# LahiruCooray/rl-aerial-manipulator

Hardware: AMD Instinct MI355X
Metric: env-steps/sec (whole node), hexacopter+arm waypoint task at 4096 envs/GPU (higher is better)
Workload: dtype f32

## Files before the change

### rl-aerial-manipulator_amd/csrc/amenv_capi.hip

```cpp
#include <hip/hip_runtime.h>
#include <hip/hip_ext.h>

#include <algorithm>
#include <cmath>
#include <cstdio>
#include <cstdlib>
#include <cstring>
#include <mutex>
#include <new>
#include <string>
#include <vector>

#include "amenv_kernels.hpp"
#include "amenv_team.hpp"
#include "amenv_team_host.hpp"
#include "amenv_quad.hpp"
#include "amenv_team_policy.hpp"
#include "amenv_quad_policy.hpp"
#include "amenv_lane_policy.hpp"
#include "amenv_rigid_policy.hpp"
#include "amenv_obsnorm.hpp"
#include "amenv_policy.hpp"
#include "amenv_train.hpp"
#include "amenv_mlp_train.hpp"
// ... 10 lines not shown
  TwoWave,
};

struct amenv {
  amenv_config cfg;
  int device = -1;
  int obs_dim = 20, act_dim = kActDim, nf = 0;
  void* blob = nullptr;
  unsigned long long* stats = nullptr;
  size_t blob_bytes = 0, fbytes = 0, ibytes = 0;
  uint32_t tile_bytes = 0;
  int n_tiles = 0;
  int block = 64;
  StepFamily family = StepFamily::Lane;
  void* team_consts = nullptr;
  uint32_t* pol_pack = nullptr;
  int pub_nj = 0;
  float* io_act = nullptr;
  float* io_obs = nullptr;
  float* io_term = nullptr;
  uint64_t steps = 0;
  bool dr = false;
  DrRanges dr_r = {{1.0f, 1.0f, 1.0f}, {0.0f, 0.0f, 0.0f}};
  bool lag = false;
  double lag_a[2] = {1.0, 1.0};
  void* lag_w = nullptr;
  hipEvent_t ev_start = nullptr, ev_stop = nullptr;
  std::string err;
  std::string kname;
};
// ... 334 lines not shown
  const amenv_config& c = e.cfg;
  const char* t = c.dtype == AMENV_F64 ? "double" : "float";
  const int nrot = (c.vehicle.n_rotors == 4 || c.vehicle.n_rotors == 6) ? c.vehicle.n_rotors : AMENV_MAX_ROTORS;
  const int kw = is_v1(&c) ? 2 : (c.task.num_waypoints == 1 ? 1 : AMENV_MAX_WAYPOINTS);
  char buf[200] = "";
  switch (e.family) {
    case StepFamily::Lane:
      std::snprintf(buf, sizeof(buf), "step_kernel<%s,NROT=%d,KW=%d,%s> block=%d", t, nrot, kw, c.vehicle.n_joints ? "v2+arm3" : (is_v1(&c) ? "v1" : "v2"), e.block); break;
    case StepFamily::LaneHelper:
      std::snprintf(buf, sizeof(buf), "step_kernel_pw<%s,NROT=%d,KW=%d,%s> (main wave + reset wave [+ observation wave + Monitor wave] per 64-env tile)", t, nrot, kw,
                    is_v1(&c) ? "v1" : "v2"); break;
    case StepFamily::Quad:
      std::snprintf(buf, sizeof(buf), "step_kernel_quad<NROT=%d,v2> (4 lanes per env, 16 envs per wave + episode-end helper wave)", c.vehicle.n_rotors); break;
    case StepFamily::Team:
      std::snprintf(buf, sizeof(buf), "step_kernel_team<%s,NROT=6,v2+arm3> (16 lanes per env: 4 RK4 stages x 4 components, 4 envs per wave + %s)", t,
                    team_wide(e) ? "one episode-end helper wave per 4" : "episode-end helper wave"); break;
    case StepFamily::Staged:
      std::snprintf(buf, sizeof(buf), "step_kernel_armk<%s,NROT=6> block=320 (4 RK4 stage waves + main wave per 64-env tile)", t); break;
    case StepFamily::TwoWave:
      std::snprintf(buf, sizeof(buf), "step_kernel_arm2w<float,NROT=6> block=128 (2 waves per 64-env tile)"); break;
  }
  std::string name = buf;
  if (e.dr) name += " +dr";
  if (e.lag) name += " +lag";
  if (e.pub_nj == 1 || e.pub_nj == 2) name += " [" + std::to_string(e.pub_nj) + "-joint arm: phantom links inside, pack / unpack at the C ABI]";
  return name;
}

template <typename... P, typename... A>
hipError_t launch(const amenv& e, bool timed, void (*k)(P...), dim3 grid, dim3 block, size_t lds, hipStream_t s, A... args) {
  if (timed) hipExtLaunchKernelGGL(k, grid, block, lds, s, e.ev_start, e.ev_stop, 0, args...);
// ... 32 lines not shown
hipError_t launch_step(const amenv& e, const StepIO& io, int T_steps, hipStream_t s, bool timed) {
  if (T_steps > 0) return launch_rollout<T, NROT, KW, VAR, NJ, DR, LAG>(e, io, T_steps, s);
  ArmArg<T, NJ> AA;
  if constexpr (NJ > 0) AA.p = make_arm<T>(e); else AA.unused = 0;
  const HotParams<T, NROT> P = make_hot<T, NROT>(e);
  const ColdParams C = make_cold(e);
  const StepTail tl{io.terminal_obs, io.ep_return, io.ep_len, io.stats};
  const uint32_t tb = e.tile_bytes;
  const int32_t n = e.cfg.num_envs;
  switch (e.family) {
    case StepFamily::Team:
      if constexpr (NJ == 3 && !DR) {
        const TeamParamsT<T> TP = make_team<T>(e);
        if (team_wide(e))
          return launch(e, timed, step_kernel_team<T, NROT, 4>, dim3(e.n_tiles * 4), dim3(320), 0, s, e.blob, n, int32_t(e.n_tiles * 4),
                        reinterpret_cast<const float*>(io.actions), TP.consts, io.obs, static_cast<T*>(io.reward), io.done, io.info, tl, C);
        return launch(e, timed, step_kernel_team<T, NROT, 1>, dim3(e.n_tiles * 16), dim3(128), 0, s, e.blob, n, int32_t(e.n_tiles * 16),
                      reinterpret_cast<const float*>(io.actions), TP.consts, io.obs, static_cast<T*>(io.reward), io.done, io.info, tl, C);
      }
      break;
    case StepFamily::Staged:
      if constexpr (NJ == 3 && !DR) {
        if constexpr (sizeof(T) == 8) {
          hipError_t ea = hipFuncSetAttribute(reinterpret_cast<const void*>(&step_kernel_armk<T, NROT>), hipFuncAttributeMaxDynamicSharedMemorySize, 96 * 1024);
          if (ea != hipSuccess) return ea;
        }
        const size_t lds = size_t(64 * ObsDim<VAR, NJ>::value + 12 * 64) * sizeof(float) + size_t((4 * kAggSlots + 6) * 64) * sizeof(T);
        return launch(e, timed, step_kernel_armk<T, NROT>, dim3(e.n_tiles), dim3(320), lds, s, e.blob, tb, n, io.actions, io.obs, io.reward, io.done, io.info, tl, P, C, AA);
      }
      break;
    case StepFamily::TwoWave:
      if constexpr (NJ == 3 && sizeof(T) == 4 && !DR) {
        const size_t lds = size_t(64 * ObsDim<VAR, NJ>::value + (kArmXchgSlots + 12) * 64) * sizeof(float);
// ... 59 lines not shown
}

template <typename T>
hipError_t launch_observe(const amenv& e, float* obs, float* ee, hipStream_t s) {
  const int n = e.cfg.num_envs, bs = 256, K = e.cfg.task.num_waypoints, nj = e.cfg.vehicle.n_joints;
  if (obs) hipLaunchKernelGGL((observe_kernel<T>), dim3((n + bs - 1) / bs), dim3(bs), 0, s, n, K, e.cfg.task.variant, nj, e.cfg.task.ee_task, e.tile_bytes, make_arm<T>(e),
                              (const void*)e.blob, obs);
  if (ee) hipLaunchKernelGGL((ee_position_kernel<T>), dim3((n + bs - 1) / bs), dim3(bs), 0, s, n, K, nj, e.tile_bytes, make_arm<T>(e), (const void*)e.blob, ee);
  return hipGetLastError();
}

template <typename T>
hipError_t launch_transpose(const amenv& e, void* f, int32_t* i, int to_api, hipStream_t s) {
  const int bs = 256, n = e.cfg.num_envs;
  hipLaunchKernelGGL((transpose_state_kernel<T>), dim3((n + bs - 1) / bs), dim3(bs), 0, s, n, e.nf, e.cfg.task.num_waypoints, e.pub_nj , e.tile_bytes, e.blob, (T*)f, i, to_api);
  return hipGetLastError();
}

bool aligned16(const void* p) { return (reinterpret_cast<uintptr_t>(p) & 15u) == 0; }

#ifndef AMENV_RIGID_WG16_MAX
#define AMENV_RIGID_WG16_MAX 6144
#endif
#ifndef AMENV_RIGID_WG64_MAX
#define AMENV_RIGID_WG64_MAX 24576
#endif
template <int NROT, int KW, int VAR, bool NORM, bool DR, bool LAG>
hipError_t launch_rigid_policy_k(const amenv& e, int T, const PolicyIO& io, const NormArg& N, hipStream_t s) {
  const HotParams<float, NROT> HP = make_hot<float, NROT>(e);
  const ColdParams C = make_cold(e);
// ... 270 lines not shown
  };
  DeviceGuard g(device);
  hipError_t s;
  if ((s = hipMalloc(&e->blob, e->blob_bytes)) != hipSuccess ||
      (s = hipMalloc((void**)&e->stats, sizeof(unsigned long long) * kStatsWords)) != hipSuccess ||
      (s = hipMemset(e->blob, 0, e->blob_bytes)) != hipSuccess ||
      (s = hipMemset(e->stats, 0, sizeof(unsigned long long) * kStatsWords)) != hipSuccess ||
      (s = (cfg->dtype == AMENV_F64 ? launch_reset<double>(*e, nullptr, nullptr, 1, nullptr) : launch_reset<float>(*e, nullptr, nullptr, 1, nullptr))) != hipSuccess ||
      (s = hipDeviceSynchronize()) != hipSuccess)
    return alloc_failed("device allocation failed", s);
  const bool quad = quad_ok(*cfg), team = team_ok(*cfg);
  if (rigid_pol_ok(*cfg) || arm_pol_ok(*cfg))
    if ((s = hipMalloc((void**)&e->pol_pack, size_t(kPolPackWords) * sizeof(uint32_t))) != hipSuccess) return alloc_failed("policy pack", s);
  if ((quad || team) && (s = upload_team_consts<float>(e, team)) != hipSuccess) return alloc_failed(quad ? "quad constants" : "team constants", s);
  if (family == StepFamily::Team && cfg->dtype == AMENV_F64 && (s = upload_team_consts<double>(e, true)) != hipSuccess) return alloc_failed("team constants (fp64)", s);
  if (e->pub_nj == 1 || e->pub_nj == 2) {
    if ((s = hipMalloc((void**)&e->io_act, n * 7 * sizeof(float))) != hipSuccess || (s = hipMalloc((void**)&e->io_obs, n * 29 * sizeof(float))) != hipSuccess ||
        (s = hipMalloc((void**)&e->io_term, n * 29 * sizeof(float))) != hipSuccess)
      return alloc_failed("n-link adapter buffers", s);
  }
  *out = e;
  return AMENV_OK;
}

int amenv_destroy(amenv* e) {
  if (!e) return AMENV_OK;
  {
    DeviceGuard g(e->device);
    if (e->blob) (void)hipFree(e->blob);
    if (e->stats) (void)hipFree(e->stats);
    if (e->team_consts) (void)hipFree(e->team_consts);
    if (e->pol_pack) (void)hipFree(e->pol_pack);
    if (e->lag_w) (void)hipFree(e->lag_w);
    if (e->io_act) (void)hipFree(e->io_act);
    if (e->io_obs) (void)hipFree(e->io_obs);
    if (e->io_term) (void)hipFree(e->io_term);
    if (e->ev_start) (void)hipEventDestroy(e->ev_start);
    if (e->ev_stop) (void)hipEventDestroy(e->ev_stop);
  }
  delete e;
  return AMENV_OK;
}

const char* amenv_last_error(const amenv* e) { return e ? e->err.c_str() : g_create_err.c_str(); }
const char* amenv_kernel_name(const amenv* e) { return e ? e->kname.c_str() : ""; }

// ... 1 lines not shown
hipError_t pad_actions(const amenv& e, const float* actions, hipStream_t s) {
  const int n = e.cfg.num_envs;
  hipLaunchKernelGGL(arm_pad_actions_kernel, dim3((n * 7 + 255) / 256), dim3(256), 0, s, actions, n, e.pub_nj, e.io_act);
  return hipGetLastError();
}
hipError_t cut_obs(const amenv& e, const float* rows29, const uint8_t* rows_of, float* out, hipStream_t s) {
  const int n = e.cfg.num_envs, od = 23 + 2 * e.pub_nj;
  hipLaunchKernelGGL(arm_cut_obs_kernel, dim3((n * od + 255) / 256), dim3(256), 0, s, rows29, n, e.pub_nj, rows_of, out);
  return hipGetLastError();
}
}

int amenv_set_seed(amenv* e, uint64_t seed) {
  if (!e) return AMENV_ERR_INVALID;
  e->cfg.seed = seed;
  return AMENV_OK;
}

int amenv_set_randomization(amenv* e, const amenv_randomization* r) {
  if (!e) return AMENV_ERR_INVALID;
  if (!r) {
    e->dr = false;
    e->dr_r = DrRanges{{1.0f, 1.0f, 1.0f}, {0.0f, 0.0f, 0.0f}};
    e->kname = kernel_name(*e);
    return AMENV_OK;
  }
  if (r->struct_size != sizeof(amenv_randomization)) return fail(e, AMENV_ERR_INVALID, "amenv_set_randomization: struct_size must be sizeof(amenv_randomization)");
  if (e->cfg.vehicle.n_joints > 0)
    return fail(e, AMENV_ERR_INVALID, "amenv_set_randomization: built for rigid vehicles (an arm vehicle's mass and inertia are not one scalar scale)");
  if (e->cfg.vehicle.n_rotors != 4 && e->cfg.vehicle.n_rotors != 6)
// ... 89 lines not shown
  if (!in) return fail(e, AMENV_ERR_INVALID, "amenv_set_rotor_state: NULL argument");
  if (!e->lag) return fail(e, AMENV_ERR_INVALID, "amenv_set_rotor_state: the rotor lag is off (amenv_set_rotor_lag)");
  DeviceGuard g(e->device);
  hipStream_t s = (hipStream_t)stream;
  AMENV_HIP(e, e->cfg.dtype == AMENV_F64 ? launch_lag_transpose<double>(*e, const_cast<void*>(in), 0, s) : launch_lag_transpose<float>(*e, const_cast<void*>(in), 0, s));
  return AMENV_OK;
}

int amenv_reset(amenv* e, const uint8_t* mask, float* obs_out, void* stream) {
  if (!e) return AMENV_ERR_INVALID;
  DeviceGuard g(e->device);
  hipStream_t s = (hipStream_t)stream;
  float* o = (e->io_obs && obs_out) ? e->io_obs : obs_out;
  AMENV_HIP(e, e->cfg.dtype == AMENV_F64 ? launch_reset<double>(*e, mask, o, 0, s) : launch_reset<float>(*e, mask, o, 0, s));
  if (e->lag) AMENV_HIP(e, e->cfg.dtype == AMENV_F64 ? launch_lag_reset<double>(*e, mask, s) : launch_lag_reset<float>(*e, mask, s));
  if (o != obs_out) AMENV_HIP(e, cut_obs(*e, e->io_obs, nullptr, obs_out, s));
  return AMENV_OK;
}

int amenv_observe(amenv* e, float* obs_out, void* stream) {
  if (!e || !obs_out) return fail(e, AMENV_ERR_INVALID, "amenv_observe: NULL argument");
  DeviceGuard g(e->device);
  hipStream_t s = (hipStream_t)stream;
  float* o = e->io_obs ? e->io_obs : obs_out;
  AMENV_HIP(e, e->cfg.dtype == AMENV_F64 ? launch_observe<double>(*e, o, nullptr, s) : launch_observe<float>(*e, o, nullptr, s));
  if (o != obs_out) AMENV_HIP(e, cut_obs(*e, e->io_obs, nullptr, obs_out, s));
  return AMENV_OK;
}

int amenv_ee_position(amenv* e, float* ee_out, void* stream) {
// ... 41 lines not shown
  return AMENV_OK;
}

int amenv_rollout(amenv* e, int32_t n_steps, const float* actions, float* obs, void* reward, uint8_t* done, uint32_t* info_bits,
                  void* stream) {
  if (!e) return AMENV_ERR_INVALID;
  if (n_steps <= 0 || !actions) return fail(e, AMENV_ERR_INVALID, "amenv_rollout: n_steps must be > 0 and actions non-NULL");
  if (!aligned16(actions) || (obs && !aligned16(obs))) return fail(e, AMENV_ERR_INVALID, "amenv_rollout: actions/obs must be 16-byte aligned");
  if (e->family == StepFamily::Team && e->cfg.dtype == AMENV_F64) return fail(e, AMENV_ERR_INVALID, "amenv_rollout: the fp64 lane-team build is a logic gate of amenv_step only");
  if (e->io_act) return fail(e, AMENV_ERR_INVALID, "amenv_rollout: arms with 1 or 2 joints are served through amenv_step (the adapters at the C ABI are per step)");
  DeviceGuard g(e->device);
  StepIO io{reinterpret_cast<const float4*>(actions), obs, reward, done, info_bits, nullptr, nullptr, nullptr, e->stats};
  hipStream_t s = (hipStream_t)stream;
  hipError_t st = e->cfg.dtype == AMENV_F64 ? dispatch_step<double>(*e, io, n_steps, s) : dispatch_step<float>(*e, io, n_steps, s);
  AMENV_HIP(e, st);
  e->steps += uint64_t(e->cfg.num_envs) * uint64_t(n_steps);
  return AMENV_OK;
}

int amenv_rollout_policy(amenv* e, int32_t n_steps, const float* flat_params, uint64_t seed, uint32_t draw0, float* obs, float* actions, float* logp,
                         float* values, float* rewards, uint8_t* dones, uint32_t* info_bits, float* terminal_obs, void* stream) {
  if (!e) return AMENV_ERR_INVALID;
  const bool quad = !e->dr && !e->lag && quad_ok(e->cfg), rigid = !quad && rigid_pol_ok(e->cfg);
  if (!quad && !rigid && !arm_pol_ok(e->cfg))
    return fail(e, AMENV_ERR_INVALID, "amenv_rollout_policy: built for fp32 vehicles: rigid with 4 or 6 rotors (every task), or the 6-rotor vehicle with a "
                "1..3-link arm (v2 task, 1..4 waypoints, any joint axes)");
  if (n_steps <= 0 || !flat_params || !obs || !actions || !logp || !values || !rewards || !dones)
    return fail(e, AMENV_ERR_INVALID, "amenv_rollout_policy: n_steps must be > 0 and flat_params / obs / actions / logp / values / rewards / dones non-NULL");
  if (rigid && (!aligned16(obs) || !aligned16(actions) || (terminal_obs && !aligned16(terminal_obs))))
    return fail(e, AMENV_ERR_INVALID, "amenv_rollout_policy: obs / actions / terminal_obs must be 16-byte aligned");
// ... 4 lines not shown
  if (quad) {
    const QuadParams QP = make_quad(*e);
    const dim3 gq(e->n_tiles * 4), bq(256);
    if (e->cfg.vehicle.n_rotors == 4) hipLaunchKernelGGL((rollout_policy_kernel_quad<4>), gq, bq, 0, s, e->blob, e->tile_bytes, n, (int)n_steps, io, e->stats, make_cold(*e), QP);
    else hipLaunchKernelGGL((rollout_policy_kernel_quad<6>), gq, bq, 0, s, e->blob, e->tile_bytes, n, (int)n_steps, io, e->stats, make_cold(*e), QP);
  } else if (rigid) {
    AMENV_HIP(e, launch_rigid_policy<false>(*e, (int)n_steps, io, NormArg{nullptr, 0.0f, 0.0, 0}, s));
  } else if (e->family == StepFamily::Team && !e->io_act) {
    const TeamParams TP = make_team<float>(*e);
    if (n <= 4096) hipLaunchKernelGGL((rollout_policy_kernel_team<6, 1>), dim3(e->n_tiles * 4), dim3(256), 0, s, e->blob, e->tile_bytes, n, (int)n_steps, io, e->stats, make_cold(*e), TP);
    else hipLaunchKernelGGL((rollout_policy_kernel_team<6, 2>), dim3(e->n_tiles * 4), dim3(256), 0, s, e->blob, e->tile_bytes, n, (int)n_steps, io, e->stats, make_cold(*e), TP);
  } else {
    AMENV_HIP(e, launch_lane_policy(*e, (int)n_steps, io, s));
  }
  AMENV_HIP(e, hipGetLastError());
  e->steps += uint64_t(e->cfg.num_envs) * uint64_t(n_steps);
  return AMENV_OK;
}

int amenv_get_state(amenv* e, void* fstate, int32_t* istate, void* stream) {
  if (!e) return AMENV_ERR_INVALID;
  DeviceGuard g(e->device);
  hipStream_t s = (hipStream_t)stream;
  AMENV_HIP(e, e->cfg.dtype == AMENV_F64 ? launch_transpose<double>(*e, fstate, istate, 1, s) : launch_transpose<float>(*e, fstate, istate, 1, s));
  return AMENV_OK;
}

int amenv_set_state(amenv* e, const void* fstate, const int32_t* istate, void* stream) {
  if (!e) return AMENV_ERR_INVALID;
  DeviceGuard g(e->device);
  hipStream_t s = (hipStream_t)stream;
  AMENV_HIP(e, e->cfg.dtype == AMENV_F64 ? launch_transpose<double>(*e, const_cast<void*>(fstate), const_cast<int32_t*>(istate), 0, s)
                                          : launch_transpose<float>(*e, const_cast<void*>(fstate), const_cast<int32_t*>(istate), 0, s));
  return AMENV_OK;
}

int amenv_stats_read(amenv* e, amenv_stats* out, int reset, void* stream) {
  if (!e || !out) return fail(e, AMENV_ERR_INVALID, "amenv_stats_read: NULL argument");
  DeviceGuard g(e->device);
  hipStream_t s = (hipStream_t)stream;
  static_assert(S_COUNT <= kStatsStride, "stats replica stride");
  std::vector<unsigned long long> rep(size_t(kStatsReplicas) * kStatsStride);
  AMENV_HIP(e, hipMemcpyAsync(rep.data(), e->stats, rep.size() * sizeof(unsigned long long), hipMemcpyDeviceToHost, s));
  if (reset) AMENV_HIP(e, hipMemsetAsync(e->stats, 0, rep.size() * sizeof(unsigned long long), s));
  AMENV_HIP(e, hipStreamSynchronize(s));
  unsigned long long h[S_COUNT] = {0};
  for (int r = 0; r < kStatsReplicas; r++)
    for (int k = 0; k < S_COUNT; k++) h[k] += rep[size_t(r) * kStatsStride + k];
// ... 391 lines not shown
```

### rl-aerial-manipulator_amd/csrc/amenv_team.hpp

```cpp
#pragma once
#include <type_traits>

#include "amenv_kernels.hpp"

#define AMENV_FN __device__ __forceinline__

namespace amenv_dev {

template <int CTRL> __device__ __forceinline__ float dpp_(float v) {
  return __builtin_bit_cast(float, __builtin_amdgcn_update_dpp(0, __builtin_bit_cast(int, v), CTRL, 0xF, 0xF, true));
}
template <int CTRL> __device__ __forceinline__ double dpp_(double v) {
  const int lo = __builtin_amdgcn_update_dpp(0, __double2loint(v), CTRL, 0xF, 0xF, true);
  const int hi = __builtin_amdgcn_update_dpp(0, __double2hiint(v), CTRL, 0xF, 0xF, true);
  return __hiloint2double(hi, lo);
}
template <int P0, int P1, int P2, int P3> __device__ __forceinline__ float qp(float v) { return dpp_<P0 | (P1 << 2) | (P2 << 4) | (P3 << 6)>(v); }
template <int P0, int P1, int P2, int P3> __device__ __forceinline__ double qp(double v) { return dpp_<P0 | (P1 << 2) | (P2 << 4) | (P3 << 6)>(v); }
template <int P0, int P1, int P2, int P3> __device__ __forceinline__ int qpi(int v) {
  return __builtin_amdgcn_update_dpp(0, v, P0 | (P1 << 2) | (P2 << 4) | (P3 << 6), 0xF, 0xF, true);
}
template <int N> __device__ __forceinline__ float row_ror(float v) { return dpp_<0x120 + N>(v); }
template <int N> __device__ __forceinline__ double row_ror(double v) { return dpp_<0x120 + N>(v); }
template <int N> __device__ __forceinline__ float row_shr(float v) { return dpp_<0x110 + N>(v); }
// ... 56 lines not shown
#pragma unroll
      for (int k = 0; k < NC4; k++) {
        const float4 v = tab[k * 16 + (lane & 15)];
        c[4 * k] = v.x; c[4 * k + 1] = v.y; c[4 * k + 2] = v.z; c[4 * k + 3] = v.w;
      }
    } else {
      const X* tab = static_cast<const X*>(table);
#pragma unroll
      for (int k = 0; k < NC4 * 4; k++) c[k] = tab[k * 16 + (lane & 15)];
    }
  }
};
using TeamLane = TeamLaneT<float>;

template <typename X>
__device__ __forceinline__ void team_load_issue(const char* tile, int i, const TeamLaneT<X>& L, TeamEnvT<X>& E) {
  constexpr uint32_t GB = 64u * 4u * sizeof(X);
  const uint32_t eoff = (uint32_t(i & 63) * 4u + uint32_t(L.cc)) * uint32_t(sizeof(X));
  auto gload = [&](int g) { return *reinterpret_cast<const X*>(tile + kIntBytes + uint32_t(g) * GB + eoff); };
  E.y = TeamStateT<X>{gload(0), gload(1), gload(2), gload(3), gload(5), gload(6)};
  E.WP = gload(4);
  const int4 iv = *(reinterpret_cast<const int4*>(tile) + (i & 63));
  E.step = iv.x; E.counter = iv.y; E.flags = iv.z; E.episode = iv.w;
}
template <typename X>
__device__ __forceinline__ void team_load_unpack(TeamEnvT<X>& E) {
  E.final_yaw = bc<3>(E.y.P); E.last_distance = bc<3>(E.y.V); E.ep_return = bc<3>(E.y.W);
}
template <typename X>
__device__ __forceinline__ void team_load(const char* tile, int i, const TeamLaneT<X>& L, TeamEnvT<X>& E) {
  team_load_issue(tile, i, L, E);
  team_load_unpack(E);
}

template <typename X>
__device__ __forceinline__ void team_store(char* tile, int i, const TeamLaneT<X>& L, const TeamEnvT<X>& E, bool store_wp = true) {
  constexpr uint32_t GB = 64u * 4u * sizeof(X);
  const uint32_t eoff = (uint32_t(i & 63) * 4u + uint32_t(L.cc)) * uint32_t(sizeof(X));
// ... 150 lines not shown
template <typename S> __device__ __forceinline__ S team_scalar_load(const void* p) {
  typedef const __attribute__((address_space(4))) uint32_t ConstWord;
  ConstWord* src = (ConstWord*)p;
  S v;
  uint32_t* dst = reinterpret_cast<uint32_t*>(&v);
  static_assert(sizeof(S) % 4 == 0, "copied word by word");
#pragma unroll
  for (int k = 0; k < int(sizeof(S) / 4); k++) dst[k] = src[k];
  return v;
}
template <typename X> __device__ __forceinline__ TeamParamsT<X> team_load_params(const void* block) {
  return team_scalar_load<TeamParamsT<X>>(static_cast<const char*>(block) + team_table_bytes<X>());
}
__device__ __forceinline__ const void* team_launder(const void* p) { asm volatile("" : "+s"(p)); return p; }

template <typename X> struct TeamStepLateArgs { float* obs; X* reward_out; uint8_t* done; uint32_t* info; StepTail tl; ColdParams C; };
struct TeamStepFirstArgs { void* blob; int32_t n_envs, n_blocks; const float* actions; const void* lane_consts; };
template <typename X> using TeamStepKernelFn = void (*)(decltype(TeamStepFirstArgs::blob), decltype(TeamStepFirstArgs::n_envs), decltype(TeamStepFirstArgs::n_blocks),
                                                        decltype(TeamStepFirstArgs::actions), decltype(TeamStepFirstArgs::lane_consts), decltype(TeamStepLateArgs<X>::obs),
                                                        decltype(TeamStepLateArgs<X>::reward_out), decltype(TeamStepLateArgs<X>::done), decltype(TeamStepLateArgs<X>::info),
                                                        decltype(TeamStepLateArgs<X>::tl), decltype(TeamStepLateArgs<X>::C));
template <typename X> __device__ __forceinline__ TeamStepLateArgs<X> team_late_args() {
  static_assert(sizeof(TeamStepFirstArgs) == 32 && alignof(TeamStepLateArgs<X>) == 8 && alignof(StepTail) == 8 && alignof(ColdParams) == 8,
                "TeamStepLateArgs mirrors the argument segment from byte 32 on");
  const void* ka = team_launder((const void*)__builtin_amdgcn_kernarg_segment_ptr());
  struct Head { float* obs; X* reward_out; uint8_t* done; uint32_t* info; StepTail tl; };
  static_assert(sizeof(Head) == offsetof(TeamStepLateArgs<X>, C), "the arguments in front of ColdParams");
  const Head h = team_scalar_load<Head>(static_cast<const char*>(ka) + sizeof(TeamStepFirstArgs));
  TeamStepLateArgs<X> a;
  a.obs = h.obs; a.reward_out = h.reward_out; a.done = h.done; a.info = h.info; a.tl = h.tl;
  return a;
}
template <typename X> __device__ __forceinline__ ColdParams team_late_cold() {
  const void* ka = team_launder((const void*)__builtin_amdgcn_kernarg_segment_ptr());
  return team_scalar_load<ColdParams>(static_cast<const char*>(ka) + sizeof(TeamStepFirstArgs) + offsetof(TeamStepLateArgs<X>, C));
}

template <typename X, int NROT, int MW>
__global__ __launch_bounds__(64 * (MW + 1)) void step_kernel_team(void* __restrict__ blob, int32_t n_envs, int32_t n_blocks, const float* __restrict__ actions,
                                                        const void* __restrict__ lane_consts, float* __restrict__ obs, X* __restrict__ reward_out,
                                                        uint8_t* __restrict__ done, uint32_t* __restrict__ info, const StepTail tl, const ColdParams C) {
  constexpr uint32_t tile_bytes = kIntBytes + 7u * 64u * 4u * uint32_t(sizeof(X));
  static_assert(NROT == 6, "team kernel: 6-rotor airframe");
  constexpr int AD = 7, OD = 29;
  __shared__ X rst[3][64];
  static_assert(MW == 1 || MW == 4, "one helper wave of 64 lanes = 16 quads serves at most four integrating waves");
  constexpr int ROWS = 4 * MW;
  __shared__ uint32_t fl[ROWS][4];
  __shared__ uint32_t have[ROWS];
  __shared__ unsigned long long acc[S_COUNT];
#ifdef AMENV_STAMPS
  unsigned long long stamps_[kStampSlots] = {0, 0, 0, 0, 0, 0, 0, 0};
#endif
  const int wave = __builtin_amdgcn_readfirstlane(int(threadIdx.x) >> 6);
  const int role = wave == MW ? 1 : 0;
  team_arg(blob, n_envs, n_blocks, actions, lane_consts);
  AMENV_STAMP(0);
  TeamLaneT<X> L;
  L.init_lane();
  const int row = role ? L.lane >> 2 : wave * 4 + (L.lane >> 4);
  const int i0 = (MW == 1 ? team_group_of_block(int(blockIdx.x), n_blocks) : team_group16_of_block(int(blockIdx.x), n_blocks)) * ROWS;
  const int i = i0 + row;
  const bool active = i < n_envs;
  char* tile = static_cast<char*>(blob) + size_t(i0 >> 6) * tile_bytes;
  TeamEnvT<X> E;
#ifdef AMENV_TEAM_DIAG_NOHELPER
  if (role == 1) { __syncthreads(); return; }
#endif
  if (role == 1) {
    {
      constexpr uint32_t GB = 64u * 4u * sizeof(X);
      const uint32_t eoff = (uint32_t(i & 63) * 4u + uint32_t(L.cc)) * uint32_t(sizeof(X));
      E.y.P = *reinterpret_cast<const X*>(tile + kIntBytes + eoff);
      E.y.V = *reinterpret_cast<const X*>(tile + kIntBytes + GB + eoff);
      const int4 iv = *(reinterpret_cast<const int4*>(tile) + (i & 63));
      E.step = iv.x; E.counter = iv.y; E.flags = iv.z; E.episode = iv.w;
    }
    const TeamParamsT<X> P = team_load_params<X>(team_launder(lane_consts));
    const X ce[3] = {L.cc == 0 ? X(1) : X(0), L.cc == 1 ? X(1) : X(0), L.cc == 2 ? X(1) : X(0)};
    static_assert(TC_E0 == 0 && TC_E1 == 1 && TC_E2 == 2, "ce[] stands in for c[] in team_reset_draw");
    const bool owned = n_blocks <= kStatsReplicas;
    if (L.lane < S_COUNT) acc[L.lane] = 0ull;
    const X dtc = P.h * X(P.substeps), slack = X(0.01) + X(50) * dtc * dtc;
    const X reach = fma_(dtc, abs_(E.y.V), abs_(E.y.P)) + slack;
    const bool lane_may = (L.cc < 3 && !(reach < X(5.7735))) || (L.cc == 2 && !(E.y.P - dtc * abs_(E.y.V) - slack > X(0.1)));
    const unsigned long long mm = __ballot(lane_may);
#ifdef AMENV_TEAM_DIAG_NOPREDICT
    constexpr bool kPredict = false;
#else
    constexpr bool kPredict = true;
#endif
    const bool serve = row < ROWS;
    const bool hlead = serve && L.cc == 0;
    const bool may = kPredict && serve && (((mm >> (L.lane & 60)) & 0xFull) != 0ull || E.step >= P.max_steps || ((E.flags & AMENV_FLAGBIT_FWR) && E.counter >= P.counter_limit) ||
                                  (P.flags & AMENV_FLAG_NAN_GUARD));
    if (hlead) have[row] = may ? 1u : 0u;
    unsigned long long* totals = tl.stats + size_t(blockIdx.x & (kStatsReplicas - 1)) * kStatsStride;
    unsigned long long mine = 0ull;
    bool fetched = false;
    if (__ballot(may) != 0ull) {
      if (owned && L.lane < S_COUNT) mine = totals[L.lane];
      fetched = true;
      if (may) {
        const TeamResetT<X> R = team_reset_draw<X>(C, ce, L.cc, E.episode, i);
        rst[0][L.lane] = R.P; rst[1][L.lane] = R.WP; rst[2][L.lane] = R.final_yaw;
      }
    }
    __syncthreads();
#ifdef AMENV_TEAM_DIAG_NOPOST
    return;
#endif
    const bool ended = hlead && (fl[hlead ? row : 0][0] & 1u) != 0;
    if (__ballot(ended) != 0ull) {
      if (!fetched && owned && L.lane < S_COUNT) mine = totals[L.lane];
      if (ended) {
        const uint32_t bits = fl[row][1];
        const int ep_len = int(fl[row][2]);
        const float ep_ret = __uint_as_float(fl[row][3]);
        if (tl.ep_return) tl.ep_return[i] = ep_ret;
        if (tl.ep_len) tl.ep_len[i] = ep_len;
        if (owned) accumulate_stats_lane(acc, 0, bits, ep_len, ep_ret);
        else accumulate_stats_lane(tl.stats, int(blockIdx.x), bits, ep_len, ep_ret);
      }
      if (owned) {
        __builtin_amdgcn_fence(__ATOMIC_ACQ_REL, "wavefront");
        __builtin_amdgcn_wave_barrier();
        if (L.lane < S_COUNT) totals[L.lane] = mine + acc[L.lane];
      }
    }
    return;
  }
#ifndef AMENV_TEAM_DIAG_NOPRIO
  __builtin_amdgcn_s_setprio(3);
#endif
  const int ia = active ? i : n_envs - 1;
  team_load_issue(tile, i, L, E);
  const float act_f = actions[size_t(ia) * AD + L.cc];
  const float actj_f = actions[size_t(ia) * AD + 4 + (L.cc < 3 ? L.cc : 2)];
  L.load_table(lane_consts);
  __builtin_amdgcn_sched_barrier(0);
  const TeamParamsT<X> P = team_load_params<X>(team_launder(lane_consts));
  const TeamStepLateArgs<X> A = team_late_args<X>();
  __builtin_amdgcn_sched_barrier(0);
  L.init_obs_cols();
  const ColdParams Cm{};
  team_load_unpack(E);
  const X act = X(act_f), actj = X(actj_f);
  const uint32_t obs_bytes = uint32_t(n_envs) * uint32_t(OD * 4);
  const uint32_t rowb = uint32_t(i) * uint32_t(OD * 4);
  uint32_t voA = L.okA ? rowb + L.offA * 4u : kOob, voB = L.okB ? rowb + L.offB * 4u : kOob, voC = L.okC ? rowb + L.offC * 4u : kOob;
  asm volatile("" : "+v"(voA), "+v"(voB), "+v"(voC));
  const __amdgpu_buffer_rsrc_t r_obs = team_rsrc(A.obs, obs_bytes), r_term = team_rsrc(A.tl.terminal_obs, A.tl.terminal_obs ? obs_bytes : 0u);
  uint32_t so1 = 0, so2 = 0, voR = kOob, voD = kOob;
  if constexpr (sizeof(X) == 4) {
    constexpr uint32_t GB = 64u * 4u * 4u;
    const uint32_t eoff = (uint32_t(i & 63) * 4u + uint32_t(L.cc)) * 4u;
    so1 = kIntBytes + uint32_t(L.bb) * GB + eoff;
    so2 = L.q2 ? eoff : kIntBytes + (L.q0 ? 5u : (L.q1 ? 6u : 4u)) * GB + eoff;
    voR = active && L.lead ? uint32_t(i) * 4u : kOob; voD = active && L.lead ? uint32_t(i) : kOob;
    asm volatile("" : "+v"(so1), "+v"(so2), "+v"(voR), "+v"(voD));
  }
  AMENV_STAMP(1);
  AMENV_STAMP_DRAIN();
  AMENV_STAMP(2);
  TeamOutT<X> o = team_advance<NROT, true>(P, Cm, L, E, act, actj, i, active, nullptr, nullptr, nullptr);
  const bool resets = o.ended && (P.flags & AMENV_FLAG_AUTO_RESET);
  if (L.lead) {
    fl[row][0] = (o.ended && active ? 1u : 0u) | (resets ? 2u : 0u);
    if (o.ended) { fl[row][1] = o.bits; fl[row][2] = uint32_t(o.ep_len); fl[row][3] = __float_as_uint(o.ep_ret); }
  }
  AMENV_STAMP(4);
#ifdef AMENV_STAMPS
  stamps_[3] = __ballot(o.ended && active) != 0ull ? 1ull : 0ull;
#endif
  __syncthreads();
  const bool any_end = __ballot(o.ended) != 0ull;
  const X tA = o.vA, tB = o.vB, tC = o.vC;
  if (any_end && resets) {
    TeamResetT<X> R;
    const int hl = row * 4 + L.cc;
    if (have[row]) R = TeamResetT<X>{rst[0][hl], rst[1][hl], rst[2][hl], X(0), X(0), X(0)};
    else R = team_reset_draw<X>(team_late_cold<X>(), L.c, L.cc, E.episode, i);
    team_apply_reset(L, team_reset_obs(P, L, R), E, o);
  }
  AMENV_STAMP(5);
  if constexpr (sizeof(X) == 4) {
    const __amdgpu_buffer_rsrc_t r_tile = team_rsrc(tile, tile_bytes);
    const bool l3 = L.cc == 3;
    const X g0 = sel(l3, E.final_yaw, E.y.P), g1 = sel(l3, E.last_distance, E.y.V), g3 = sel(l3, E.ep_return, E.y.W);
    const X sv = sel(L.q0, g0, sel(L.q1, g1, sel(L.q2, E.y.Q, g3)));
    __builtin_amdgcn_raw_buffer_store_b32(__float_as_int(sv), r_tile, int(so1), 0, 0);
    const int ival = sel(L.cc == 0, E.step, sel(L.cc == 1, E.counter, sel(L.cc == 2, E.flags, E.episode)));
    const float s2 = sel(L.q0, E.y.TH, sel(L.q1, E.y.THD, sel(L.q2, __int_as_float(ival), E.WP)));
    __builtin_amdgcn_raw_buffer_store_b32(__float_as_int(s2), r_tile, int(L.bb == 3 && !resets ? kOob : so2), 0, 0);
  } else {
    team_store(tile, i, L, E, resets);
  }
  __builtin_amdgcn_raw_buffer_store_b32(__float_as_int(float(o.vA)), r_obs, int(voA), 0, 0);
  __builtin_amdgcn_raw_buffer_store_b32(__float_as_int(float(o.vB)), r_obs, int(voB), 0, 0);
  __builtin_amdgcn_raw_buffer_store_b32(__float_as_int(float(o.vC)), r_obs, int(voC), 0, 0);
  if constexpr (sizeof(X) == 4) {
    const uint32_t nb = uint32_t(n_envs);
    __builtin_amdgcn_raw_buffer_store_b32(__float_as_int(o.reward), team_rsrc(A.reward_out, nb * 4u), int(voR), 0, 0);
    __builtin_amdgcn_raw_buffer_store_b8(uint8_t(o.ended ? 1 : 0), team_rsrc(A.done, nb), int(voD), 0, 0);
    __builtin_amdgcn_raw_buffer_store_b32(int(o.bits), team_rsrc(A.info, nb * 4u), int(voR), 0, 0);
  } else {
    if (active && L.lead) { A.reward_out[uint32_t(i)] = o.reward; A.done[uint32_t(i)] = o.ended ? 1 : 0; A.info[uint32_t(i)] = o.bits; }
  }
  if (any_end) {
    __builtin_amdgcn_raw_buffer_store_b32(__float_as_int(float(tA)), r_term, int(o.ended ? voA : kOob), 0, 0);
    __builtin_amdgcn_raw_buffer_store_b32(__float_as_int(float(tB)), r_term, int(o.ended ? voB : kOob), 0, 0);
    __builtin_amdgcn_raw_buffer_store_b32(__float_as_int(float(tC)), r_term, int(o.ended ? voC : kOob), 0, 0);
  }
  AMENV_STAMP(6);
#ifdef AMENV_STAMPS
  AMENV_STAMP_DRAIN();
  AMENV_STAMP(7);
  if (L.lane == 0 && blockIdx.x * MW + wave < kStampWaves)
    for (int kk = 0; kk < kStampSlots; kk++) A.tl.stats[kStampBase + (blockIdx.x * MW + wave) * kStampSlots + kk] = stamps_[kk];
#endif
}

static_assert(std::is_same<decltype(&step_kernel_team<float, 6, 4>), TeamStepKernelFn<float>>::value && std::is_same<decltype(&step_kernel_team<float, 6, 1>), TeamStepKernelFn<float>>::value &&
                  std::is_same<decltype(&step_kernel_team<double, 6, 4>), TeamStepKernelFn<double>>::value && std::is_same<decltype(&step_kernel_team<double, 6, 1>), TeamStepKernelFn<double>>::value,
              "step_kernel_team's parameters and TeamStepFirstArgs / TeamStepLateArgs have come apart");

template <int NROT>
// ... 30 lines not shown
```

Measured before the change: 945.3 million.

## Replace team helper-wave reset draws with a persistent reset-draw cache

Adds a per-env device cache of precomputed reset draws keyed by episode parity. The helper wave now only refills the next episode's entry when it is stale. The integrating waves read the cached draw instead of waiting at a __syncthreads for LDS results from the helper. Episode statistics and ep_return/ep_len writes move into the main waves as atomics. This removes the block barrier and the helper's predictive draw and stats work. In exchange it adds global cache traffic, refresh kernels and memsets after reset, step and state loads, and atomics on episode end.

```diff
diff --git a/rl-aerial-manipulator_amd/csrc/amenv_capi.hip b/rl-aerial-manipulator_amd/csrc/amenv_capi.hip
--- a/rl-aerial-manipulator_amd/csrc/amenv_capi.hip
+++ b/rl-aerial-manipulator_amd/csrc/amenv_capi.hip
@@ -48,6 +48,7 @@
   int block = 64;
   StepFamily family = StepFamily::Lane;
   void* team_consts = nullptr;
+  void* team_rcache = nullptr;
   uint32_t* pol_pack = nullptr;
   int pub_nj = 0;
   float* io_act = nullptr;
@@ -412,7 +413,7 @@
       std::snprintf(buf, sizeof(buf), "step_kernel_quad<NROT=%d,v2> (4 lanes per env, 16 envs per wave + episode-end helper wave)", c.vehicle.n_rotors); break;
     case StepFamily::Team:
       std::snprintf(buf, sizeof(buf), "step_kernel_team<%s,NROT=6,v2+arm3> (16 lanes per env: 4 RK4 stages x 4 components, 4 envs per wave + %s)", t,
-                    team_wide(e) ? "one episode-end helper wave per 4" : "episode-end helper wave"); break;
+                    team_wide(e) ? "one reset-cache keeper wave per 4" : "reset-cache keeper wave"); break;
     case StepFamily::Staged:
       std::snprintf(buf, sizeof(buf), "step_kernel_armk<%s,NROT=6> block=320 (4 RK4 stage waves + main wave per 64-env tile)", t); break;
     case StepFamily::TwoWave:
@@ -475,9 +476,9 @@
         const TeamParamsT<T> TP = make_team<T>(e);
         if (team_wide(e))
           return launch(e, timed, step_kernel_team<T, NROT, 4>, dim3(e.n_tiles * 4), dim3(320), 0, s, e.blob, n, int32_t(e.n_tiles * 4),
-                        reinterpret_cast<const float*>(io.actions), TP.consts, io.obs, static_cast<T*>(io.reward), io.done, io.info, tl, C);
+                        reinterpret_cast<const float*>(io.actions), TP.consts, e.team_rcache, io.obs, static_cast<T*>(io.reward), io.done, io.info, tl, C);
         return launch(e, timed, step_kernel_team<T, NROT, 1>, dim3(e.n_tiles * 16), dim3(128), 0, s, e.blob, n, int32_t(e.n_tiles * 16),
-                      reinterpret_cast<const float*>(io.actions), TP.consts, io.obs, static_cast<T*>(io.reward), io.done, io.info, tl, C);
+                      reinterpret_cast<const float*>(io.actions), TP.consts, e.team_rcache, io.obs, static_cast<T*>(io.reward), io.done, io.info, tl, C);
       }
       break;
     case StepFamily::Staged:
@@ -567,6 +568,18 @@
 hipError_t launch_transpose(const amenv& e, void* f, int32_t* i, int to_api, hipStream_t s) {
   const int bs = 256, n = e.cfg.num_envs;
   hipLaunchKernelGGL((transpose_state_kernel<T>), dim3((n + bs - 1) / bs), dim3(bs), 0, s, n, e.nf, e.cfg.task.num_waypoints, e.pub_nj , e.tile_bytes, e.blob, (T*)f, i, to_api);
+  return hipGetLastError();
+}
+
+hipError_t team_rcache_refresh(const amenv& e, hipStream_t s) {
+  if (!e.team_rcache) return hipSuccess;
+  const bool f64 = e.cfg.dtype == AMENV_F64;
+  const int n_pad = e.n_tiles * 64;
+  hipError_t st = hipMemsetAsync(e.team_rcache, kResetCacheStale, size_t(n_pad) * kResetCacheWords * (f64 ? 8 : 4), s);
+  if (st != hipSuccess) return st;
+  const dim3 grid((n_pad * 4 + 255) / 256), block(256);
+  if (f64) hipLaunchKernelGGL(team_rcache_fill_kernel<double>, grid, block, 0, s, (const void*)e.blob, e.tile_bytes, n_pad, static_cast<double*>(e.team_rcache), make_cold(e));
+  else hipLaunchKernelGGL(team_rcache_fill_kernel<float>, grid, block, 0, s, (const void*)e.blob, e.tile_bytes, n_pad, static_cast<float*>(e.team_rcache), make_cold(e));
   return hipGetLastError();
 }
 
@@ -867,6 +880,11 @@
     if ((s = hipMalloc((void**)&e->pol_pack, size_t(kPolPackWords) * sizeof(uint32_t))) != hipSuccess) return alloc_failed("policy pack", s);
   if ((quad || team) && (s = upload_team_consts<float>(e, team)) != hipSuccess) return alloc_failed(quad ? "quad constants" : "team constants", s);
   if (family == StepFamily::Team && cfg->dtype == AMENV_F64 && (s = upload_team_consts<double>(e, true)) != hipSuccess) return alloc_failed("team constants (fp64)", s);
+  if (family == StepFamily::Team) {
+    if ((s = hipMalloc(&e->team_rcache, size_t(e->n_tiles) * 64 * kResetCacheWords * ts)) != hipSuccess || (s = team_rcache_refresh(*e, nullptr)) != hipSuccess ||
+        (s = hipDeviceSynchronize()) != hipSuccess)
+      return alloc_failed("team reset-draw cache", s);
+  }
   if (e->pub_nj == 1 || e->pub_nj == 2) {
     if ((s = hipMalloc((void**)&e->io_act, n * 7 * sizeof(float))) != hipSuccess || (s = hipMalloc((void**)&e->io_obs, n * 29 * sizeof(float))) != hipSuccess ||
         (s = hipMalloc((void**)&e->io_term, n * 29 * sizeof(float))) != hipSuccess)
@@ -883,6 +901,7 @@
     if (e->blob) (void)hipFree(e->blob);
     if (e->stats) (void)hipFree(e->stats);
     if (e->team_consts) (void)hipFree(e->team_consts);
+    if (e->team_rcache) (void)hipFree(e->team_rcache);
     if (e->pol_pack) (void)hipFree(e->pol_pack);
     if (e->lag_w) (void)hipFree(e->lag_w);
     if (e->io_act) (void)hipFree(e->io_act);
@@ -914,6 +933,12 @@
 int amenv_set_seed(amenv* e, uint64_t seed) {
   if (!e) return AMENV_ERR_INVALID;
   e->cfg.seed = seed;
+  if (e->team_rcache) {
+    DeviceGuard g(e->device);
+    AMENV_HIP(e, hipDeviceSynchronize());
+    AMENV_HIP(e, hipMemset(e->team_rcache, kResetCacheStale, size_t(e->n_tiles) * 64 * kResetCacheWords * (e->cfg.dtype == AMENV_F64 ? 8 : 4)));
+    AMENV_HIP(e, hipDeviceSynchronize());
+  }
   return AMENV_OK;
 }
 
@@ -1033,6 +1058,7 @@
   float* o = (e->io_obs && obs_out) ? e->io_obs : obs_out;
   AMENV_HIP(e, e->cfg.dtype == AMENV_F64 ? launch_reset<double>(*e, mask, o, 0, s) : launch_reset<float>(*e, mask, o, 0, s));
   if (e->lag) AMENV_HIP(e, e->cfg.dtype == AMENV_F64 ? launch_lag_reset<double>(*e, mask, s) : launch_lag_reset<float>(*e, mask, s));
+  AMENV_HIP(e, team_rcache_refresh(*e, s));
   if (o != obs_out) AMENV_HIP(e, cut_obs(*e, e->io_obs, nullptr, obs_out, s));
   return AMENV_OK;
 }
@@ -1104,6 +1130,7 @@
   hipStream_t s = (hipStream_t)stream;
   hipError_t st = e->cfg.dtype == AMENV_F64 ? dispatch_step<double>(*e, io, n_steps, s) : dispatch_step<float>(*e, io, n_steps, s);
   AMENV_HIP(e, st);
+  AMENV_HIP(e, team_rcache_refresh(*e, s));
   e->steps += uint64_t(e->cfg.num_envs) * uint64_t(n_steps);
   return AMENV_OK;
 }
@@ -1138,6 +1165,7 @@
     AMENV_HIP(e, launch_lane_policy(*e, (int)n_steps, io, s));
   }
   AMENV_HIP(e, hipGetLastError());
+  AMENV_HIP(e, team_rcache_refresh(*e, s));
   e->steps += uint64_t(e->cfg.num_envs) * uint64_t(n_steps);
   return AMENV_OK;
 }
@@ -1156,6 +1184,7 @@
   hipStream_t s = (hipStream_t)stream;
   AMENV_HIP(e, e->cfg.dtype == AMENV_F64 ? launch_transpose<double>(*e, const_cast<void*>(fstate), const_cast<int32_t*>(istate), 0, s)
                                           : launch_transpose<float>(*e, const_cast<void*>(fstate), const_cast<int32_t*>(istate), 0, s));
+  AMENV_HIP(e, team_rcache_refresh(*e, s));
   return AMENV_OK;
 }
 
diff --git a/rl-aerial-manipulator_amd/csrc/amenv_team.hpp b/rl-aerial-manipulator_amd/csrc/amenv_team.hpp
--- a/rl-aerial-manipulator_amd/csrc/amenv_team.hpp
+++ b/rl-aerial-manipulator_amd/csrc/amenv_team.hpp
@@ -94,14 +94,22 @@
 using TeamLane = TeamLaneT<float>;
 
 template <typename X>
-__device__ __forceinline__ void team_load_issue(const char* tile, int i, const TeamLaneT<X>& L, TeamEnvT<X>& E) {
+__device__ __forceinline__ void team_load_issue_ints(const char* tile, int i, TeamEnvT<X>& E) {
+  const int4 iv = *(reinterpret_cast<const int4*>(tile) + (i & 63));
+  E.step = iv.x; E.counter = iv.y; E.flags = iv.z; E.episode = iv.w;
+}
+template <typename X>
+__device__ __forceinline__ void team_load_issue_state(const char* tile, int i, const TeamLaneT<X>& L, TeamEnvT<X>& E) {
   constexpr uint32_t GB = 64u * 4u * sizeof(X);
   const uint32_t eoff = (uint32_t(i & 63) * 4u + uint32_t(L.cc)) * uint32_t(sizeof(X));
   auto gload = [&](int g) { return *reinterpret_cast<const X*>(tile + kIntBytes + uint32_t(g) * GB + eoff); };
   E.y = TeamStateT<X>{gload(0), gload(1), gload(2), gload(3), gload(5), gload(6)};
   E.WP = gload(4);
-  const int4 iv = *(reinterpret_cast<const int4*>(tile) + (i & 63));
-  E.step = iv.x; E.counter = iv.y; E.flags = iv.z; E.episode = iv.w;
+}
+template <typename X>
+__device__ __forceinline__ void team_load_issue(const char* tile, int i, const TeamLaneT<X>& L, TeamEnvT<X>& E) {
+  team_load_issue_state(tile, i, L, E);
+  team_load_issue_ints(tile, i, E);
 }
 template <typename X>
 __device__ __forceinline__ void team_load_unpack(TeamEnvT<X>& E) {
@@ -282,15 +290,41 @@
 }
 __device__ __forceinline__ const void* team_launder(const void* p) { asm volatile("" : "+s"(p)); return p; }
 
+constexpr int kResetCacheWords = 16;
+constexpr int kResetCacheStale = 0xFF;
+__device__ __forceinline__ float team_rcache_tag(float, int32_t episode) { return __int_as_float(episode); }
+__device__ __forceinline__ double team_rcache_tag(double, int32_t episode) { return double(episode); }
+__device__ __forceinline__ bool team_rcache_hit(float tag, int32_t episode) { return __float_as_int(tag) == episode; }
+__device__ __forceinline__ bool team_rcache_hit(double tag, int32_t episode) { return tag == double(episode); }
+__device__ __forceinline__ uint32_t team_rcache_slot(int i, int32_t episode) { return (uint32_t(i) * 2u + uint32_t(episode & 1)) * 8u; }
+template <typename X>
+__device__ __forceinline__ void team_rcache_store(X* __restrict__ rc, int i, int cc, int32_t episode, const TeamResetT<X>& R) {
+  X* s = rc + team_rcache_slot(i, episode);
+  s[cc] = cc == 3 ? R.final_yaw : R.P;
+  s[4 + cc] = cc == 3 ? team_rcache_tag(X(0), episode) : R.WP;
+}
+static_assert(TC_E0 == 0 && TC_E1 == 1 && TC_E2 == 2, "team_unit_consts stands in for c[] in team_reset_draw");
+template <typename X> __device__ __forceinline__ void team_unit_consts(int cc, X (&ce)[3]) { ce[0] = cc == 0 ? X(1) : X(0); ce[1] = cc == 1 ? X(1) : X(0); ce[2] = cc == 2 ? X(1) : X(0); }
+template <typename X>
+__global__ __launch_bounds__(256) void team_rcache_fill_kernel(const void* __restrict__ blob, uint32_t tile_bytes, int32_t n_pad, X* __restrict__ rc, const ColdParams C) {
+  const int t = int(blockIdx.x * blockDim.x + threadIdx.x), i = t >> 2, cc = t & 3;
+  if (i >= n_pad) return;
+  const int32_t episode = (reinterpret_cast<const int4*>(tile_base(blob, tile_bytes, i)) + (i & 63))->w;
+  X ce[3];
+  team_unit_consts(cc, ce);
+#pragma unroll
+  for (int k = 0; k < 2; k++) team_rcache_store(rc, i, cc, episode + k, team_reset_draw<X>(C, ce, cc, episode + k, i));
+}
+
 template <typename X> struct TeamStepLateArgs { float* obs; X* reward_out; uint8_t* done; uint32_t* info; StepTail tl; ColdParams C; };
-struct TeamStepFirstArgs { void* blob; int32_t n_envs, n_blocks; const float* actions; const void* lane_consts; };
+struct TeamStepFirstArgs { void* blob; int32_t n_envs, n_blocks; const float* actions; const void* lane_consts; void* rcache; };
 template <typename X> using TeamStepKernelFn = void (*)(decltype(TeamStepFirstArgs::blob), decltype(TeamStepFirstArgs::n_envs), decltype(TeamStepFirstArgs::n_blocks),
-                                                        decltype(TeamStepFirstArgs::actions), decltype(TeamStepFirstArgs::lane_consts), decltype(TeamStepLateArgs<X>::obs),
-                                                        decltype(TeamStepLateArgs<X>::reward_out), decltype(TeamStepLateArgs<X>::done), decltype(TeamStepLateArgs<X>::info),
-                                                        decltype(TeamStepLateArgs<X>::tl), decltype(TeamStepLateArgs<X>::C));
+                                                        decltype(TeamStepFirstArgs::actions), decltype(TeamStepFirstArgs::lane_consts), decltype(TeamStepFirstArgs::rcache),
+                                                        decltype(TeamStepLateArgs<X>::obs), decltype(TeamStepLateArgs<X>::reward_out), decltype(TeamStepLateArgs<X>::done),
+                                                        decltype(TeamStepLateArgs<X>::info), decltype(TeamStepLateArgs<X>::tl), decltype(TeamStepLateArgs<X>::C));
 template <typename X> __device__ __forceinline__ TeamStepLateArgs<X> team_late_args() {
-  static_assert(sizeof(TeamStepFirstArgs) == 32 && alignof(TeamStepLateArgs<X>) == 8 && alignof(StepTail) == 8 && alignof(ColdParams) == 8,
-                "TeamStepLateArgs mirrors the argument segment from byte 32 on");
+  static_assert(sizeof(TeamStepFirstArgs) == 40 && alignof(TeamStepLateArgs<X>) == 8 && alignof(StepTail) == 8 && alignof(ColdParams) == 8,
+                "TeamStepLateArgs mirrors the argument segment from byte 40 on");
   const void* ka = team_launder((const void*)__builtin_amdgcn_kernarg_segment_ptr());
   struct Head { float* obs; X* reward_out; uint8_t* done; uint32_t* info; StepTail tl; };
   static_assert(sizeof(Head) == offsetof(TeamStepLateArgs<X>, C), "the arguments in front of ColdParams");
@@ -306,23 +340,19 @@
 
 template <typename X, int NROT, int MW>
 __global__ __launch_bounds__(64 * (MW + 1)) void step_kernel_team(void* __restrict__ blob, int32_t n_envs, int32_t n_blocks, const float* __restrict__ actions,
-                                                        const void* __restrict__ lane_consts, float* __restrict__ obs, X* __restrict__ reward_out,
+                                                        const void* __restrict__ lane_consts, void* __restrict__ rcache, float* __restrict__ obs, X* __restrict__ reward_out,
                                                         uint8_t* __restrict__ done, uint32_t* __restrict__ info, const StepTail tl, const ColdParams C) {
   constexpr uint32_t tile_bytes = kIntBytes + 7u * 64u * 4u * uint32_t(sizeof(X));
   static_assert(NROT == 6, "team kernel: 6-rotor airframe");
   constexpr int AD = 7, OD = 29;
-  __shared__ X rst[3][64];
   static_assert(MW == 1 || MW == 4, "one helper wave of 64 lanes = 16 quads serves at most four integrating waves");
   constexpr int ROWS = 4 * MW;
-  __shared__ uint32_t fl[ROWS][4];
-  __shared__ uint32_t have[ROWS];
-  __shared__ unsigned long long acc[S_COUNT];
 #ifdef AMENV_STAMPS
   unsigned long long stamps_[kStampSlots] = {0, 0, 0, 0, 0, 0, 0, 0};
 #endif
   const int wave = __builtin_amdgcn_readfirstlane(int(threadIdx.x) >> 6);
   const int role = wave == MW ? 1 : 0;
-  team_arg(blob, n_envs, n_blocks, actions, lane_consts);
+  team_arg(blob, n_envs, n_blocks, actions, lane_consts, rcache);
   AMENV_STAMP(0);
   TeamLaneT<X> L;
   L.init_lane();
@@ -331,70 +361,24 @@
   const int i = i0 + row;
   const bool active = i < n_envs;
   char* tile = static_cast<char*>(blob) + size_t(i0 >> 6) * tile_bytes;
+  X* const rc = static_cast<X*>(rcache);
   TeamEnvT<X> E;
 #ifdef AMENV_TEAM_DIAG_NOHELPER
-  if (role == 1) { __syncthreads(); return; }
+  constexpr bool kCached = false;
+  if (role == 1) return;
+#else
+  constexpr bool kCached = true;
 #endif
   if (role == 1) {
-    {
-      constexpr uint32_t GB = 64u * 4u * sizeof(X);
-      const uint32_t eoff = (uint32_t(i & 63) * 4u + uint32_t(L.cc)) * uint32_t(sizeof(X));
-      E.y.P = *reinterpret_cast<const X*>(tile + kIntBytes + eoff);
-      E.y.V = *reinterpret_cast<const X*>(tile + kIntBytes + GB + eoff);
-      const int4 iv = *(reinterpret_cast<const int4*>(tile) + (i & 63));
-      E.step = iv.x; E.counter = iv.y; E.flags = iv.z; E.episode = iv.w;
-    }
-    const TeamParamsT<X> P = team_load_params<X>(team_launder(lane_consts));
-    const X ce[3] = {L.cc == 0 ? X(1) : X(0), L.cc == 1 ? X(1) : X(0), L.cc == 2 ? X(1) : X(0)};
-    static_assert(TC_E0 == 0 && TC_E1 == 1 && TC_E2 == 2, "ce[] stands in for c[] in team_reset_draw");
-    const bool owned = n_blocks <= kStatsReplicas;
-    if (L.lane < S_COUNT) acc[L.lane] = 0ull;
-    const X dtc = P.h * X(P.substeps), slack = X(0.01) + X(50) * dtc * dtc;
-    const X reach = fma_(dtc, abs_(E.y.V), abs_(E.y.P)) + slack;
-    const bool lane_may = (L.cc < 3 && !(reach < X(5.7735))) || (L.cc == 2 && !(E.y.P - dtc * abs_(E.y.V) - slack > X(0.1)));
-    const unsigned long long mm = __ballot(lane_may);
-#ifdef AMENV_TEAM_DIAG_NOPREDICT
-    constexpr bool kPredict = false;
-#else
-    constexpr bool kPredict = true;
-#endif
-    const bool serve = row < ROWS;
-    const bool hlead = serve && L.cc == 0;
-    const bool may = kPredict && serve && (((mm >> (L.lane & 60)) & 0xFull) != 0ull || E.step >= P.max_steps || ((E.flags & AMENV_FLAGBIT_FWR) && E.counter >= P.counter_limit) ||
-                                  (P.flags & AMENV_FLAG_NAN_GUARD));
-    if (hlead) have[row] = may ? 1u : 0u;
-    unsigned long long* totals = tl.stats + size_t(blockIdx.x & (kStatsReplicas - 1)) * kStatsStride;
-    unsigned long long mine = 0ull;
-    bool fetched = false;
-    if (__ballot(may) != 0ull) {
-      if (owned && L.lane < S_COUNT) mine = totals[L.lane];
-      fetched = true;
-      if (may) {
-        const TeamResetT<X> R = team_reset_draw<X>(C, ce, L.cc, E.episode, i);
-        rst[0][L.lane] = R.P; rst[1][L.lane] = R.WP; rst[2][L.lane] = R.final_yaw;
-      }
-    }
-    __syncthreads();
-#ifdef AMENV_TEAM_DIAG_NOPOST
-    return;
-#endif
-    const bool ended = hlead && (fl[hlead ? row : 0][0] & 1u) != 0;
-    if (__ballot(ended) != 0ull) {
-      if (!fetched && owned && L.lane < S_COUNT) mine = totals[L.lane];
-      if (ended) {
-        const uint32_t bits = fl[row][1];
-        const int ep_len = int(fl[row][2]);
-        const float ep_ret = __uint_as_float(fl[row][3]);
-        if (tl.ep_return) tl.ep_return[i] = ep_ret;
-        if (tl.ep_len) tl.ep_len[i] = ep_len;
-        if (owned) accumulate_stats_lane(acc, 0, bits, ep_len, ep_ret);
-        else accumulate_stats_lane(tl.stats, int(blockIdx.x), bits, ep_len, ep_ret);
-      }
-      if (owned) {
-        __builtin_amdgcn_fence(__ATOMIC_ACQ_REL, "wavefront");
-        __builtin_amdgcn_wave_barrier();
-        if (L.lane < S_COUNT) totals[L.lane] = mine + acc[L.lane];
-      }
+    if (row >= ROWS) return;
+    const X tagw = rc[size_t(i) * kResetCacheWords + 7u + 8u * uint32_t(L.cc & 1)];
+    team_load_issue_ints(tile, i, E);
+    const int32_t next = E.episode + 1;
+    const X tag = (next & 1) ? bc<1>(tagw) : bc<0>(tagw);
+    if (!team_rcache_hit(tag, next)) {
+      X ce[3];
+      team_unit_consts(L.cc, ce);
+      team_rcache_store(rc, i, L.cc, next, team_reset_draw<X>(C, ce, L.cc, next, i));
     }
     return;
   }
@@ -402,7 +386,8 @@
   __builtin_amdgcn_s_setprio(3);
 #endif
   const int ia = active ? i : n_envs - 1;
-  team_load_issue(tile, i, L, E);
+  team_load_issue_ints(tile, i, E);
+  team_load_issue_state(tile, i, L, E);
   const float act_f = actions[size_t(ia) * AD + L.cc];
   const float actj_f = actions[size_t(ia) * AD + 4 + (L.cc < 3 ? L.cc : 2)];
   L.load_table(lane_consts);
@@ -412,7 +397,6 @@
   __builtin_amdgcn_sched_barrier(0);
   L.init_obs_cols();
   const ColdParams Cm{};
-  team_load_unpack(E);
   const X act = X(act_f), actj = X(actj_f);
   const uint32_t obs_bytes = uint32_t(n_envs) * uint32_t(OD * 4);
   const uint32_t rowb = uint32_t(i) * uint32_t(OD * 4);
@@ -428,28 +412,35 @@
     voR = active && L.lead ? uint32_t(i) * 4u : kOob; voD = active && L.lead ? uint32_t(i) : kOob;
     asm volatile("" : "+v"(so1), "+v"(so2), "+v"(voR), "+v"(voD));
   }
+  __builtin_amdgcn_sched_barrier(0);
+  X cP = X(0), cW = X(0);
+  if constexpr (kCached) {
+    const X* ce = rc + team_rcache_slot(i, E.episode) + L.cc;
+    cP = ce[0]; cW = ce[4];
+  }
+  team_load_unpack(E);
   AMENV_STAMP(1);
   AMENV_STAMP_DRAIN();
   AMENV_STAMP(2);
   TeamOutT<X> o = team_advance<NROT, true>(P, Cm, L, E, act, actj, i, active, nullptr, nullptr, nullptr);
   const bool resets = o.ended && (P.flags & AMENV_FLAG_AUTO_RESET);
-  if (L.lead) {
-    fl[row][0] = (o.ended && active ? 1u : 0u) | (resets ? 2u : 0u);
-    if (o.ended) { fl[row][1] = o.bits; fl[row][2] = uint32_t(o.ep_len); fl[row][3] = __float_as_uint(o.ep_ret); }
-  }
   AMENV_STAMP(4);
 #ifdef AMENV_STAMPS
   stamps_[3] = __ballot(o.ended && active) != 0ull ? 1ull : 0ull;
 #endif
-  __syncthreads();
   const bool any_end = __ballot(o.ended) != 0ull;
   const X tA = o.vA, tB = o.vB, tC = o.vC;
-  if (any_end && resets) {
-    TeamResetT<X> R;
-    const int hl = row * 4 + L.cc;
-    if (have[row]) R = TeamResetT<X>{rst[0][hl], rst[1][hl], rst[2][hl], X(0), X(0), X(0)};
-    else R = team_reset_draw<X>(team_late_cold<X>(), L.c, L.cc, E.episode, i);
-    team_apply_reset(L, team_reset_obs(P, L, R), E, o);
+  const int t_len = o.ep_len;
+  const float t_ret = o.ep_ret;
+  const uint32_t t_bits = o.bits;
+  if (any_end) {
+    const X yaw = bc<3>(cP), tag = bc<3>(cW);
+    if (resets) {
+      TeamResetT<X> R{L.cc == 3 ? X(0) : cP, L.cc == 3 ? X(0) : cW, yaw, X(0), X(0), X(0)};
+      if (!kCached || !team_rcache_hit(tag, E.episode))
+        R = team_reset_draw<X>(team_late_cold<X>(), L.c, L.cc, E.episode, i);
+      team_apply_reset(L, team_reset_obs(P, L, R), E, o);
+    }
   }
   AMENV_STAMP(5);
   if constexpr (sizeof(X) == 4) {
@@ -479,6 +470,20 @@
     __builtin_amdgcn_raw_buffer_store_b32(__float_as_int(float(tA)), r_term, int(o.ended ? voA : kOob), 0, 0);
     __builtin_amdgcn_raw_buffer_store_b32(__float_as_int(float(tB)), r_term, int(o.ended ? voB : kOob), 0, 0);
     __builtin_amdgcn_raw_buffer_store_b32(__float_as_int(float(tC)), r_term, int(o.ended ? voC : kOob), 0, 0);
+    const int k = L.lane & 15;
+    const bool mine = o.ended && active;
+    uint32_t* const mp = k == 0 ? reinterpret_cast<uint32_t*>(A.tl.ep_return) : reinterpret_cast<uint32_t*>(A.tl.ep_len);
+    if (mine && k < 2 && mp) mp[uint32_t(i)] = k == 0 ? __float_as_uint(t_ret) : uint32_t(t_len);
+#ifndef AMENV_DIAG_NO_STATS
+    const bool term = (t_bits & AMENV_INFO_TERMINATED) != 0;
+    const bool caused = (t_bits & (AMENV_INFO_SUCCESS | AMENV_INFO_CRASHED | AMENV_INFO_OOB | AMENV_INFO_NONFINITE)) != 0;
+    const int cause = (t_bits & AMENV_INFO_SUCCESS) ? S_SUCCESS : (t_bits & AMENV_INFO_CRASHED) ? S_CRASHED : (t_bits & AMENV_INFO_OOB) ? S_OOB : S_NONFINITE;
+    const long long q10 = __builtin_isfinite(t_ret) ? (long long)__builtin_rintf(t_ret * 1024.0f) : 0ll;
+    const int slot = k == 0 ? S_EPISODES : k == 1 ? (term ? S_TERMINATED : S_TRUNCATED) : k == 2 ? cause : k == 3 ? S_LENGTH : S_RETURN_Q10;
+    const unsigned long long val = k < 3 ? 1ull : k == 3 ? (unsigned long long)(long long)t_len : (unsigned long long)q10;
+    unsigned long long* totals = A.tl.stats + size_t(blockIdx.x & (kStatsReplicas - 1)) * kStatsStride;
+    if (mine && k < 5 && (k != 2 || caused)) atomicAdd(&totals[slot], val);
+#endif
   }
   AMENV_STAMP(6);
 #ifdef AMENV_STAMPS
```

Result: no change. 939.2 million (median of 2 runs) (-0.6%).
